# casinca/LLM-quest

Measured on AMD Instinct MI355X. Metric: img+tokens/sec fwd+bwd, ViT-B+Qwen3-0.6B VLM, 224px+512tok, higher is better.
Workload: dtype bf16; 1 GPU; BASELINE configs[3]: VLM early fusion, ViT-B/16 (frozen, fwd) + ffn adapter 768->3072->1024 + Qwen3-0.6B, 224x224 image + 512 text tokens (S=709), fwd+loss+bwd, no optimizer step; per_gpu_batch=160, global_batch=160, parallelism=dp1, text_mask=all ones, vision_tower_precision=bf16 MFMA operands, fp32 residual stream

## Files before the change

### llm_quest_amd/csrc/attention.hip

```cpp
#include "attn_common.h"

namespace {

template <int D>
__global__ __launch_bounds__(256, 2) void attn_fwd_kernel(int B, int S, int Hq, int Hkv, const bf16_t* __restrict__ q, int64_t ldq,
                                                          const bf16_t* __restrict__ k, int64_t ldk, const bf16_t* __restrict__ v,
                                                          int64_t ldv, bf16_t* __restrict__ o, int64_t ldo, float* __restrict__ lse,
                                                          const uint8_t* __restrict__ key_mask, int causal, float scale_log2) {
    using C = Cfg<D>;
    const int abl = causal >> 8;
    causal &= 0xff;
    __shared__ __attribute__((aligned(16))) char smem[4 * C::TILE];
    const int lane = threadIdx.x & 63;
    const int wave = __builtin_amdgcn_readfirstlane(threadIdx.x >> 6);
    const int nqb = (S + 127) / 128;
    const int vid = (abl >> 8) & 1 ? (int)blockIdx.x : xcd_chunked((int)blockIdx.x, (int)gridDim.x);
    const int qb = nqb - 1 - (vid % nqb);
    const int bh = vid / nqb;
    const int hq = bh % Hq, b = bh / Hq;
    const int hkv = hq / (Hq / Hkv);
    const int q0 = qb * 128;
    const int qg = q0 + wave * 32 + (lane & 31);
    const bool qvalid = qg < S;

// ... 636 lines not shown
                    }
                    dsv[e] = __builtin_amdgcn_exp2f(t) * (pacc[st][e] - dlt);
                    if constexpr (e % 2 == 1) dsw[st][e / 2] = pack_bf2(dsv[e - 1], dsv[e]);
                };
                static_for<PD>([&](auto g) { load(g); });
                static_for<NG>([&](auto gc) {
                    constexpr int g = gc.value;
                    load(std::integral_constant<int, g + PD>{});
                    if constexpr (g < 2 * NA) {
                        constexpr int st = g / NA, ks = (g % NA) / 2, which = g % 2;
                        if constexpr ((ATTN_ABL & 8) && ks > 0) {
                        } else if constexpr (which == 0) mfma_ownedB<OWNED, QF0 + 4 * ks, ks == 0>(sacc[st], f[g % RING]);
                        else mfma_ownedB<OWNED, OF0 + 4 * ks, ks == 0>(pacc[st], f[g % RING]);
                    } else if constexpr (!(ATTN_ABL & 4)) {
                        constexpr int h = g - 2 * NA, st = h / NC, sd = (h % NC) / DT, dt = h % DT;
                        const u32x4 w = {dsw[st][4 * sd], dsw[st][4 * sd + 1], dsw[st][4 * sd + 2], dsw[st][4 * sd + 3]};
                        constexpr int younger = NG - 1 - g < PD ? NG - 1 - g : PD;
                        mfma_owned<OWNED, 16 * dt>(tr_wait<2 * younger>(ft[g % RING]), __builtin_bit_cast(bf16x8, w));
                    }
                    if constexpr (g == NA) tiles_settle(sacc[0], pacc[0]);
                    if constexpr (g == 2 * NA) tiles_settle(sacc[1], pacc[1]);
                    if constexpr (g >= NA && g < 2 * NA) {
                        constexpr int m = g - NA, per = 16 / NA;
                        static_for<per>([&](auto i) { element(std::integral_constant<int, 0>{}, std::integral_constant<int, m * per + i.value>{}); });
                    } else if constexpr (g >= 2 * NA && g < 2 * NA + NC) {
                        constexpr int m = g - 2 * NA, per = 16 / NC;
                        static_for<per>([&](auto i) { element(std::integral_constant<int, 1>{}, std::integral_constant<int, m * per + i.value>{}); });
                    }
                    __builtin_amdgcn_sched_barrier(0);
                });
            };
            if (boundary) tile_body(std::true_type{});
            else tile_body(std::false_type{});
        }
        owned_settle<OWNED>();
        bf16_t* row = dq + ((int64_t)b * S + qg) * lddq + (int64_t)hq * D;
        static_for<DT * 4>([&](auto i) {
            constexpr int dt = i.value / 4, g4 = i.value % 4, r = 16 * dt + 4 * g4;
            const int d = dt * 32 + 8 * g4 + 4 * (lane >> 5);
            const u32x2 pk = {pack_bf2(owned_read<OWNED, r>() * scale, owned_read<OWNED, r + 1>() * scale),
                              pack_bf2(owned_read<OWNED, r + 2>() * scale, owned_read<OWNED, r + 3>() * scale)};
            if (qvalid && !(abl & 2)) *reinterpret_cast<u32x2*>(row + d) = pk;
        });
    }
}

template <int D, bool LEAN>
__global__ __launch_bounds__(256, 1) void attn_bwd_dkv_kernel(int B, int S, int Hq, int Hkv, const bf16_t* __restrict__ q, int64_t ldq,
                                                              const bf16_t* __restrict__ k, int64_t ldk, const bf16_t* __restrict__ v,
                                                              int64_t ldv, const bf16_t* __restrict__ d_o, int64_t lddo,
                                                              const float* __restrict__ lse, const float* __restrict__ delta,
                                                              bf16_t* __restrict__ dk, int64_t lddk, bf16_t* __restrict__ dv, int64_t lddv,
                                                              const uint8_t* __restrict__ key_mask, int causal, float scale, float scale_log2,
                                                              int bpw, bf16_t* __restrict__ ds_out) {
    using C = Cfg<D>;
    constexpr int KS = C::KS, DT = C::DT;
    constexpr int NA = 2 * KS, NC = 4 * DT, NG = 2 * NA + 2 * NC;
    constexpr int OWNED = 32 * DT + 8 * KS, DK0 = 16 * DT, KF0 = 32 * DT, VF0 = KF0 + 4 * KS;
    constexpr int RING = ATTN_RING, PD = ATTN_PD;
    constexpr bool UNI = C::UNI;
    constexpr int NIMG = UNI ? 2 : 4, NST = 3, STAGE = NIMG * C::TILE, PIECES = NIMG * C::PPW;
    constexpr int OIMG = (UNI ? 1 : 2) * C::TILE;
    const int abl = causal >> 8;
    causal &= 0xff;
    __shared__ __attribute__((aligned(16))) char smem[NST * STAGE + NST * 512];
    char* rowc = smem + NST * STAGE;
    const int lane = threadIdx.x & 63;
    const int wave = __builtin_amdgcn_readfirstlane(threadIdx.x >> 6);
    const int nkb = (S + 127) / 128, nchunk = (nkb + bpw - 1) / bpw;
    const int chunk = blockIdx.x % nchunk, bh = blockIdx.x / nchunk;
    const int hkv = bh % Hkv, b = bh / Hkv;
    const int rep = Hq / Hkv;
    const int kb_lo = chunk * bpw, kb_hi = min(nkb, kb_lo + bpw);
    const int nqt_all = (S + 63) / 64;
    auto qt0_of = [&](int kb) { return causal ? kb * 2 : 0; };

    int ikb = kb_lo, ih = 0, iq = 0, istage = 0;
    auto issue_next = [&]() -> bool {
        if (ikb < kb_hi && iq >= nqt_all - qt0_of(ikb)) { iq = 0; ++ih; }
        if (ikb < kb_hi && ih >= rep) { ih = 0; ++ikb; }
        if (ikb >= kb_hi) return false;
        const int hq = hkv * rep + ih;
        const int qt = qt0_of(ikb) + iq;
        char* st_ = smem + istage * STAGE;
        const bf16_t* qb_ = q + ((int64_t)b * S + (int64_t)qt * 64) * ldq + (int64_t)hq * D;
        const bf16_t* ob_ = d_o + ((int64_t)b * S + (int64_t)qt * 64) * lddo + (int64_t)hq * D;
        if constexpr (UNI) {
            dma_tile<D, IMG_UNI>(qb_, ldq, S - qt * 64, st_, wave, lane);
            dma_tile<D, IMG_UNI>(ob_, lddo, S - qt * 64, st_ + OIMG, wave, lane);
        } else {
            dma_tile<D, IMG_ROW>(qb_, ldq, S - qt * 64, st_, wave, lane);
            dma_tile<D, IMG_TR>(qb_, ldq, S - qt * 64, st_ + C::TILE, wave, lane);
            dma_tile<D, IMG_ROW>(ob_, lddo, S - qt * 64, st_ + OIMG, wave, lane);
            dma_tile<D, IMG_TR>(ob_, lddo, S - qt * 64, st_ + OIMG + C::TILE, wave, lane);
        }
        {
            const float* src = ((wave & 1) == 0 ? lse : delta) + ((int64_t)b * Hq + hq) * S + (int64_t)qt * 64;
            auto rsrc = __builtin_amdgcn_make_buffer_rsrc(const_cast<float*>(src), 0, 0x7fffffff, 0x00020000);
            const unsigned voff = qt * 64 + lane < S ? (unsigned)(lane * 4) : OOB;
            __builtin_amdgcn_raw_ptr_buffer_load_lds(rsrc, LDS_PTR(rowc + istage * 512 + (wave & 1) * 256), 4, voff, 0, 0, 0);
        }
        ++iq;
        istage = istage == NST - 1 ? 0 : istage + 1;
        return true;
    };
    [[maybe_unused]] const bool prof_on = threadIdx.x == 0;
    [[maybe_unused]] unsigned long long prof_acc[16] = {};
    [[maybe_unused]] const unsigned long long t_wg = PROF_T();
    int inflight = 0;
    inflight += issue_next();
    inflight += issue_next();

    const LaneOff<D> lo = lane_offsets<D>(lane);
    const unsigned lds0 = (unsigned)(unsigned long long)LDS_PTR(smem);
    int cstage = 0;
    int st1 = 0, st2 = 0;
    bf16x8 tk[KS], tv[KS];
    auto request_kv = [&](int kb_) {
        const int kg_ = kb_ * 128 + wave * 32 + (lane & 31);
        load_rows_frag<D>(k + (int64_t)b * S * ldk + (int64_t)hkv * D, ldk, kg_, kg_ < S, lane, tk);
        load_rows_frag<D>(v + (int64_t)b * S * ldv + (int64_t)hkv * D, ldv, kg_, kg_ < S, lane, tv);
    };
    if (kb_lo < kb_hi) request_kv(kb_lo);
    for (int kb = kb_lo; kb < kb_hi; ++kb) {
        [[maybe_unused]] const unsigned long long t_pro = PROF_T();
        const int k0 = kb * 128;
        const int kg = k0 + wave * 32 + (lane & 31);
        const bool kvalid = kg < S;
        const bool kreal = kvalid && (key_mask == nullptr || key_mask[(int64_t)b * S + kg] != 0);
        owned_zero<OWNED, 0, 32 * DT>();
        if constexpr (LEAN) {
#pragma unroll
            for (int ks = 0; ks < KS; ++ks) {
                u32x4 w = __builtin_bit_cast(u32x4, tk[ks]);
#pragma unroll
                for (int e = 0; e < 4; ++e) w[e] = pack_bf2(__uint_as_float(w[e] << 16) * scale_log2, __uint_as_float(w[e] & 0xffff0000u) * scale_log2);
                tk[ks] = __builtin_bit_cast(bf16x8, w);
            }
        }
        static_for<KS>([&](auto ks) { owned_write4<OWNED, KF0 + 4 * ks.value>(tk[ks.value]); });
        static_for<KS>([&](auto ks) { owned_write4<OWNED, VF0 + 4 * ks.value>(tv[ks.value]); });
        const int qt0 = qt0_of(kb);
        const int per_head = nqt_all - qt0;
        const int nit = per_head * rep;
        PROF_ADD(3, t_pro);
        int ch = 0, cq = -1;
        for (int it = 0; it < nit; ++it) {
            if (++cq == per_head) { cq = 0; ++ch; }
            [[maybe_unused]] const unsigned long long t_w = PROF_T();
            if (inflight >= 2) {
                if (st1 + st2 == 8) wait_vmcnt<PIECES + 1 + 8>();
                else if (st1 + st2 == 4) wait_vmcnt<PIECES + 1 + 4>();
                else wait_vmcnt<PIECES + 1>();
            } else wait_vmcnt<0>();
            st2 = st1;
            st1 = 0;
            PROF_ADD(1, t_w);
            [[maybe_unused]] const unsigned long long t_b = PROF_T();
            __builtin_amdgcn_s_barrier();
            PROF_ADD(6, t_b);
            --inflight;
            [[maybe_unused]] const unsigned long long t_i = PROF_T();
            if (!(abl & 1)) inflight += issue_next();
            PROF_ADD(7, t_i);
#if ATTN_ABL & 16
            struct BodyTimer {
                unsigned long long t0; bool on; unsigned long long* acc;
                __device__ ~BodyTimer() { if (on) { acc[2] += __builtin_readcyclecounter() - t0; acc[5] += 1; } }
            } body_timer{PROF_T(), prof_on, prof_acc};
#endif
            const int qt = qt0 + cq;
            const int qroff = cstage * STAGE, qtoff = UNI ? qroff : qroff + C::TILE, oroff = qroff + OIMG, otoff = UNI ? oroff : oroff + C::TILE;
            const float* rc = reinterpret_cast<const float*>(rowc + cstage * 512) + 4 * (lane >> 5);
            cstage = cstage == NST - 1 ? 0 : cstage + 1;
            if (causal && qt * 64 + 63 < k0 + wave * 32) continue;
            const bool boundary = (causal && qt * 64 < k0 + wave * 32 + 31) || (qt * 64 + 64 > S) || __any(!kreal);
            int vqx[KS], vox[KS], vqt[DT], vot[DT];
#pragma unroll
            for (int ks = 0; ks < KS; ++ks) {
                vqx[ks] = ((UNI ? lo.rowu : lo.row) + qroff) ^ (ks << 5);
                vox[ks] = ((UNI ? lo.rowu : lo.row) + oroff) ^ (ks << 5);
            }
#pragma unroll
            for (int dt = 0; dt < DT; ++dt) {
                vqt[dt] = (UNI ? lo.colu[dt] : lo.col[dt]) + qtoff;
                vot[dt] = (UNI ? lo.colu[dt] : lo.col[dt]) + otoff;
            }

            auto tile_body = [&](auto bc) {
                constexpr bool BOUNDARY = decltype(bc)::value;
                bf16x8 f[RING] = {};
                TrHalves ft[RING] = {};
                f32x16 sacc[2], pacc[2];
                unsigned pw[2][8] = {}, dsw[2][8] = {};
                float lsr[2][16], dlr[2][16], tt[2][16], pv[2][16], dsv[2][16];
                [[maybe_unused]] f32x16 linit[2], dinit[2];
                auto load = [&](auto gc) {
                    constexpr int g = gc.value;
                    if constexpr (ATTN_ABL & 1) return;
                    if constexpr (g < 2 * NA) {
                        constexpr int st = g / NA, ks = (g % NA) / 2, which = g % 2;
                        f[g % RING] = lds_frag(smem, which ? vox[ks] : vqx[ks], st * 32 * C::ROWB);
                    } else if constexpr (g < NG) {
                        constexpr int h = g - 2 * NA, st = h / NC, sd = (h % NC) / (2 * DT), dt = (h % (2 * DT)) / 2, which = h % 2;
                        constexpr int imm = (st * 32 + 16 * sd) * C::ROWB;
                        const int va = which ? vqt[dt] : vot[dt];
                        if constexpr (!(ATTN_ABL & 32)) tr_issue<imm, imm + 8 * C::ROWB>(ft[g % RING], lds0 + va, lds0 + (UNI ? va ^ 0x20 : va));
                    }
                };
                auto row_constants = [&](auto stc) {
                    constexpr int st = stc.value;
#pragma unroll
                    for (int g4 = 0; g4 < 4; ++g4) {
                        const f32x4 a = *reinterpret_cast<const f32x4*>(rc + st * 32 + 8 * g4);
                        const f32x4 c = *reinterpret_cast<const f32x4*>(rc + 64 + st * 32 + 8 * g4);
#pragma unroll
                        for (int e = 0; e < 4; ++e) {
                            if constexpr (LEAN) {
                                linit[st][4 * g4 + e] = a[e];
                                dinit[st][4 * g4 + e] = c[e];
                            } else {
                                lsr[st][4 * g4 + e] = a[e];
                                dlr[st][4 * g4 + e] = c[e];
                            }
                        }
                    }
                };
                auto stage = [&](auto stc, auto ec, auto kc) {
                    constexpr int st = stc.value, e = ec.value, k = kc.value;
                    if constexpr (e < 0 || e >= 16 || (ATTN_ABL & 2)) return;
                    else if constexpr (LEAN) {
                        if constexpr (k == 1 && BOUNDARY) {
                            const int qq = qt * 64 + st * 32 + acc_row(e, lane);
                            const bool masked = (causal && kg > qq) || !kreal || qq >= S;
                            sacc[st][e] = masked ? -INFINITY : sacc[st][e];
                            asm volatile("" : "+v"(sacc[st][e]));
                        } else if constexpr (k == 2) {
                            pv[st][e] = __builtin_amdgcn_exp2f(sacc[st][e]);
                            asm volatile("" : "+v"(pv[st][e]));
                        } else if constexpr (k == 3) {
                            dsv[st][e] = pacc[st][e] * pv[st][e];
                            if constexpr (e % 2 == 1) {
                                pw[st][e / 2] = pack_bf2(pv[st][e - 1], pv[st][e]);
                                dsw[st][e / 2] = pack_bf2(dsv[st][e - 1], dsv[st][e]);
                                asm volatile("" : "+v"(pw[st][e / 2]), "+v"(dsw[st][e / 2]));
                            } else {
                                asm volatile("" : "+v"(dsv[st][e]));
                            }
                        }
                    } else if constexpr (k == 0) {
                        lsr[st][e] *= LOG2E;
                        asm volatile("" : "+v"(lsr[st][e]));
                    } else if constexpr (k == 1) {
                        float t = fmaf(sacc[st][e], scale_log2, -lsr[st][e]);
                        if constexpr (BOUNDARY) {
                            const int qq = qt * 64 + st * 32 + acc_row(e, lane);
                            const bool masked = (causal && kg > qq) || !kreal || qq >= S;
                            t = masked ? -INFINITY : t;
                        }
                        tt[st][e] = t;
                        asm volatile("" : "+v"(tt[st][e]));
                    } else if constexpr (k == 2) {
                        pv[st][e] = __builtin_amdgcn_exp2f(tt[st][e]);
                        dsv[st][e] = pacc[st][e] - dlr[st][e];
                        asm volatile("" : "+v"(pv[st][e]), "+v"(dsv[st][e]));
                    } else {
                        dsv[st][e] *= pv[st][e];
                        if constexpr (e % 2 == 1) {
                            pw[st][e / 2] = pack_bf2(pv[st][e - 1], pv[st][e]);
                            dsw[st][e / 2] = pack_bf2(dsv[st][e - 1], dsv[st][e]);
                            asm volatile("" : "+v"(pw[st][e / 2]), "+v"(dsw[st][e / 2]));
                        } else {
                            asm volatile("" : "+v"(dsv[st][e]));
                        }
                    }
                };
                auto b_step = [&](auto stc, auto mc, auto perc) {
                    constexpr int m = mc.value, PER = perc.value;
                    if constexpr (m >= 0 && m < 16 / PER + 3)
                        static_for<4>([&](auto kc) {
                            static_for<PER>([&](auto i) { stage(stc, std::integral_constant<int, (m - kc.value) * PER + i.value>{}, kc); });
                        });
                };
                if constexpr (LEAN) row_constants(std::integral_constant<int, 0>{});
                static_for<PD>([&](auto g) { load(g); });
                [[maybe_unused]] unsigned long long t_seg = PROF_T();
                static_for<NG>([&](auto gc) {
                    constexpr int g = gc.value;
#if ATTN_ABL & 16
                    if constexpr (g == NA || g == 2 * NA || g == 2 * NA + NC) {
                        if (prof_on) { const unsigned long long now = __builtin_readcyclecounter(); prof_acc[8 + (g == NA ? 0 : g == 2 * NA ? 1 : 2)] += now - t_seg; t_seg = now; }
                    }
#endif
                    if constexpr (!LEAN && g == NA - 1) row_constants(std::integral_constant<int, 0>{});
                    if constexpr (LEAN && g == NA - 4) row_constants(std::integral_constant<int, 1>{});
                    load(std::integral_constant<int, g + PD>{});
                    if constexpr (g < 2 * NA) {
                        constexpr int st = g / NA, ks = (g % NA) / 2, which = g % 2;
                        if constexpr ((ATTN_ABL & 8) && ks > 0) {
                        } else if constexpr (LEAN && ks == 0) {
                            if constexpr (which == 0) mfma_ownedB_init<OWNED, KF0>(sacc[st], f[g % RING], linit[st]);
                            else mfma_ownedB_init<OWNED, VF0>(pacc[st], f[g % RING], dinit[st]);
                        } else if constexpr (which == 0) mfma_ownedB<OWNED, KF0 + 4 * ks, ks == 0>(sacc[st], f[g % RING]);
                        else mfma_ownedB<OWNED, VF0 + 4 * ks, ks == 0>(pacc[st], f[g % RING]);
                    } else if constexpr (!(ATTN_ABL & 4)) {
                        constexpr int h = g - 2 * NA, st = h / NC, sd = (h % NC) / (2 * DT), dt = (h % (2 * DT)) / 2, which = h % 2;
                        constexpr int younger = NG - 1 - g < PD ? NG - 1 - g : PD;
                        const bf16x8 fa = tr_wait<2 * younger>(ft[g % RING]);
                        if constexpr (which == 0) {
                            const u32x4 w = {pw[st][4 * sd], pw[st][4 * sd + 1], pw[st][4 * sd + 2], pw[st][4 * sd + 3]};
                            mfma_owned<OWNED, 16 * dt, false>(fa, __builtin_bit_cast(bf16x8, w));
                        } else {
                            const u32x4 w = {dsw[st][4 * sd], dsw[st][4 * sd + 1], dsw[st][4 * sd + 2], dsw[st][4 * sd + 3]};
                            mfma_owned<OWNED, DK0 + 16 * dt, false>(fa, __builtin_bit_cast(bf16x8, w));
                        }
                    }
                    if constexpr (g == NA) tiles_settle(sacc[0], pacc[0]);
                    if constexpr (g == 2 * NA) tiles_settle(sacc[1], pacc[1]);
                    static_assert(16 % NA == 0 && 16 % NC == 0 && 16 / (16 / NA) + 3 <= NA + NC / 2 && 16 / (16 / NC) + 3 <= NC + NC / 2, "B phase does not fit its gaps");
                    b_step(std::integral_constant<int, 0>{}, std::integral_constant<int, g - NA>{}, std::integral_constant<int, 16 / NA>{});
                    b_step(std::integral_constant<int, 1>{}, std::integral_constant<int, g - 2 * NA>{}, std::integral_constant<int, 16 / NC>{});
                    if constexpr (!LEAN && g == 2 * NA - 1) row_constants(std::integral_constant<int, 1>{});
                    __builtin_amdgcn_sched_barrier(0);
                });
                PROF_ADD(11, t_seg);
                if (ds_out) {
                    const int hq_ = hkv * rep + ch;
                    const int nqb_ = (S + 127) / 128;
                    char* blk = reinterpret_cast<char*>(ds_out) + ((((int64_t)b * Hq + hq_) * (2 * nqb_) + qt) * 2 * (4 * nqb_) + (kb * 4 + wave)) * 2048 + lane * 16;
                    static_for<4>([&](auto i) {
                        constexpr int st = i.value / 2, c2 = i.value % 2;
                        const u32x4 w4 = {dsw[st][4 * c2], dsw[st][4 * c2 + 1], dsw[st][4 * c2 + 2], dsw[st][4 * c2 + 3]};
                        *reinterpret_cast<u32x4*>(blk + (int64_t)st * (4 * nqb_) * 2048 + c2 * 1024) = w4;
                    });
                }
            };
            if (boundary) tile_body(std::true_type{});
            else tile_body(std::false_type{});
            st1 = ds_out != nullptr ? 4 : 0;
        }
        [[maybe_unused]] const unsigned long long t_epi = PROF_T();
        owned_settle<OWNED>();
        if (kb + 1 < kb_hi) request_kv(kb + 1);
        bf16_t* krow = dk + ((int64_t)b * S + kg) * lddk + (int64_t)hkv * D + 8 * (lane >> 5);
        bf16_t* vrow = dv + ((int64_t)b * S + kg) * lddv + (int64_t)hkv * D + 8 * (lane >> 5);
        static_for<DT * 2>([&](auto i) {
            constexpr int dt = i.value / 2, gp = i.value % 2, rv = 16 * dt + 8 * gp, rk = DK0 + rv;
            const unsigned ka0 = pack_bf2(owned_read<OWNED, rk>() * scale, owned_read<OWNED, rk + 1>() * scale), ka1 = pack_bf2(owned_read<OWNED, rk + 2>() * scale, owned_read<OWNED, rk + 3>() * scale);
            const unsigned kb0 = pack_bf2(owned_read<OWNED, rk + 4>() * scale, owned_read<OWNED, rk + 5>() * scale), kb1 = pack_bf2(owned_read<OWNED, rk + 6>() * scale, owned_read<OWNED, rk + 7>() * scale);
            const unsigned va0 = pack_bf2(owned_read<OWNED, rv>(), owned_read<OWNED, rv + 1>()), va1 = pack_bf2(owned_read<OWNED, rv + 2>(), owned_read<OWNED, rv + 3>());
            const unsigned vb0 = pack_bf2(owned_read<OWNED, rv + 4>(), owned_read<OWNED, rv + 5>()), vb1 = pack_bf2(owned_read<OWNED, rv + 6>(), owned_read<OWNED, rv + 7>());
            const auto k0s = __builtin_amdgcn_permlane32_swap(ka0, kb0, false, false), k1s = __builtin_amdgcn_permlane32_swap(ka1, kb1, false, false);
            const auto v0s = __builtin_amdgcn_permlane32_swap(va0, vb0, false, false), v1s = __builtin_amdgcn_permlane32_swap(va1, vb1, false, false);
            const u32x4 wk = {k0s[0], k1s[0], k0s[1], k1s[1]}, wv = {v0s[0], v1s[0], v0s[1], v1s[1]};
            if (kvalid && !(abl & 2)) {
                *reinterpret_cast<u32x4*>(krow + dt * 32 + 16 * gp) = wk;
                *reinterpret_cast<u32x4*>(vrow + dt * 32 + 16 * gp) = wv;
            }
        });
        PROF_ADD(4, t_epi);
    }
    PROF_ADD(0, t_wg);
#if ATTN_ABL & 16
    if (prof_on)
        for (int i = 0; i < 16; ++i) atomicAdd(&g_prof[i], prof_acc[i]);
#endif
}

struct QkFuse {
    const bf16_t* qkv;
    int64_t ldqkv;
    const bf16_t* qw;
    const float* cosT;
    const float* sinT;
    const int32_t* pos;
    const float* rstd;
    int rstd_heads;
    bf16_t* dqkv;
    int64_t lddqkv;
    float* dwp;
    const bf16_t* cs16;
};
__device__ __forceinline__ void unpack4(const u32x2 v, float (&o)[4]) {
    o[0] = __uint_as_float(v[0] << 16);
    o[1] = __uint_as_float(v[0] & 0xffff0000u);
    o[2] = __uint_as_float(v[1] << 16);
    o[3] = __uint_as_float(v[1] & 0xffff0000u);
}
__device__ __forceinline__ float round_bf(float x) { return bf2f(f2bf(x)); }

#ifndef DQ_ABL
#define DQ_ABL 0
#endif
#if DQ_ABL & 16
__device__ unsigned long long g_dq_prof[32];
#define DQ_T() __builtin_readcyclecounter()
#define DQ_MARK(i) do { const unsigned long long now_ = __builtin_readcyclecounter(); dqp[i] += now_ - dq_t; dq_t = now_; } while (0)
#else
#define DQ_T() 0ull
#define DQ_MARK(i) do { } while (0)
#endif
template <int D, bool FUSE>
__global__ __launch_bounds__(256, 2) void attn_bwd_dq_spill_kernel(int B, int S, int Hq, int Hkv, const bf16_t* __restrict__ k, int64_t ldk,
                                                                   const bf16_t* __restrict__ ds, bf16_t* __restrict__ dq, int64_t lddq,
                                                                   int causal, float scale, QkFuse f) {
    using C = Cfg<D>;
    constexpr int DT = C::DT, DSW = 4096;
    constexpr int KST = 2, DST = 3, DS_BASE = KST * C::TILE, DS_STAGE = 4 * DSW;
    __shared__ __attribute__((aligned(16))) char smem[KST * C::TILE + DST * DS_STAGE];
    const int lane = threadIdx.x & 63;
    const int wave = __builtin_amdgcn_readfirstlane(threadIdx.x >> 6);
    const int nqb = (S + 127) / 128;
    const int vid = xcd_chunked((int)blockIdx.x, (int)gridDim.x);
    int qb, bh;
    heavy_first(vid, nqb, B * Hq, ATTN_HEAD_GROUP, qb, bh);
    const int hq = bh % Hq, b = bh / Hq;
    const int hkv = hq / (Hq / Hkv);
    const int q0 = qb * 128;
    const int qw = q0 + wave * 32;
    const int qg = qw + (lane & 31);
    const int ntiles_all = (S + 63) / 64;
    const int ntiles = causal ? min(ntiles_all, (q0 + 127) / 64 + 1) : ntiles_all;
    const bf16_t* kbase = k + (int64_t)b * S * ldk + (int64_t)hkv * D;
    const char* sblk = reinterpret_cast<const char*>(ds) + (((((int64_t)b * Hq + hq) * (2 * nqb) + 2 * qb + (wave >> 1)) * 2 + (wave & 1)) * (4 * nqb)) * 2048;
    auto srsrc = __builtin_amdgcn_make_buffer_rsrc(const_cast<char*>(sblk), 0, 0x7fffffff, 0x00020000);
    const unsigned unit = (unsigned)(lane ^ ((lane >> 5) << 2)) * 16;
    auto fetched = [&](int kgrp) { return !(causal && kgrp * 32 > qw + 31) && kgrp * 32 < S; };
    auto issue_k = [&](int kt) {
        if (!((DQ_ABL & 2) && kt > 0)) dma_tile<D, IMG_TR>(kbase + (int64_t)kt * 64 * ldk, ldk, S - kt * 64, smem + (kt % KST) * C::TILE, wave, lane);
    };
    auto issue_ds = [&](int kt) {
        char* mine = smem + DS_BASE + (kt % DST) * DS_STAGE + wave * DSW;
#pragma unroll
        for (int half = 0; half < 2; ++half) {
            const bool live = fetched(2 * kt + half) && kt < ntiles && !((DQ_ABL & 1) && kt > 0);
            const unsigned o0 = live ? (unsigned)((2 * kt + half) * 2048) + unit : OOB;
            const unsigned o1 = live ? (unsigned)((2 * kt + half) * 2048 + 1024) + unit : OOB;
            __builtin_amdgcn_raw_ptr_buffer_load_lds(srsrc, LDS_PTR(mine + half * 2048), 16, o0, 0, 0, 0);
            __builtin_amdgcn_raw_ptr_buffer_load_lds(srsrc, LDS_PTR(mine + half * 2048 + 1024), 16, o1, 0, 0, 0);
        }
    };
    const LaneOff<D> lok = lane_offsets<D>(lane);
    const int g = lane >> 4, q4 = (lane >> 2) & 3, p = lane & 3;
    const unsigned scol = (unsigned)((g & 1) * 1024 + ((((p & 1) * 32 + 4 * (g >> 1) + q4) ^ ((p & 1) << 2)) * 16) + (p >> 1) * 8) + DS_BASE + wave * DSW;
    const unsigned lds0 = (unsigned)(unsigned long long)LDS_PTR(smem);
    f32x16 acc[DT];
#pragma unroll
    for (int i = 0; i < DT; ++i)
#pragma unroll
        for (int e = 0; e < 16; ++e) acc[i][e] = 0.f;
    [[maybe_unused]] unsigned long long dqp[8] = {};
    [[maybe_unused]] unsigned long long dq_t = DQ_T();
    [[maybe_unused]] const unsigned long long dq_t0 = dq_t;
    [[maybe_unused]] int pos_pre[4] = {0, 0, 0, 0};
    if constexpr (FUSE) {
#pragma unroll
        for (int it = 0; it < 4; ++it) {
            const int qrow = q0 + (int)(threadIdx.x >> 3) + 32 * it;
            pos_pre[it] = f.pos[(int64_t)b * S + (qrow < S ? qrow : S - 1)];
        }
    }
    issue_ds(0);
    issue_k(0);
    issue_ds(1);
    for (int kt = 0; kt < ntiles; ++kt) {
        wait_vmcnt<4>();
        DQ_MARK(0);
        __builtin_amdgcn_s_barrier();
        DQ_MARK(1);
        if (kt + 1 < ntiles) issue_k(kt + 1);
        else issue_ds(ntiles);
        issue_ds(kt + 2);
        DQ_MARK(2);
        const unsigned kimg = lds0 + (kt % KST) * C::TILE, simg = lds0 + (kt % DST) * DS_STAGE + scol;
        static_for<2>([&](auto hc) {
            constexpr int half = hc.value;
            if (!fetched(2 * kt + half)) return;
            if constexpr (DQ_ABL & 4) return;
            TrHalves bs[2], ak[2][DT];
            static_for<2>([&](auto sc) {
// ... 343 lines not shown
    if (D == 128)
        hipLaunchKernelGGL(attn_fwd_kernel<128>, dim3((unsigned)grid), dim3(256), 0, s, B, S, Hq, Hkv, (const bf16_t*)q, ldq, (const bf16_t*)k, ldk, (const bf16_t*)v, ldv, (bf16_t*)o, ldo, lse, key_mask, causal, sl2);
    else
        hipLaunchKernelGGL(attn_fwd_kernel<64>, dim3((unsigned)grid), dim3(256), 0, s, B, S, Hq, Hkv, (const bf16_t*)q, ldq, (const bf16_t*)k, ldk, (const bf16_t*)v, ldv, (bf16_t*)o, ldo, lse, key_mask, causal, sl2);
    MI355_LAUNCH_CHECK("mi355_attn_fwd");
    return 0;
}

static int64_t attn_bwd_ds_bytes(int B, int S, int Hq) {
    const int64_t nqb = (S + 127) / 128;
    return (int64_t)B * Hq * nqb * nqb * 128 * 128 * 2;
}
extern "C" int64_t mi355_attn_bwd_workspace_bytes(int B, int S, int Hq, int D) {
    if (D != 128 || B <= 0 || S <= 0 || Hq <= 0) return 0;
    return attn_bwd_ds_bytes(B, S, Hq) + 2 * (((int64_t)B * Hq * S * 4 + 15) & ~(int64_t)15);
}

extern "C" int mi355_attn_bwd_ws(int B, int S, int Hq, int Hkv, int D, const void* q, int64_t ldq, const void* k, int64_t ldk,
                                 const void* v, int64_t ldv, const void* o, int64_t ldo, const void* d_o, int64_t lddo,
                                 const float* lse, float* delta, void* dq, int64_t lddq, void* dk, int64_t lddk, void* dv,
                                 int64_t lddv, const uint8_t* key_mask, int causal, float scale, void* workspace, int64_t workspace_bytes,
                                 void* stream);

extern "C" int mi355_attn_bwd(int B, int S, int Hq, int Hkv, int D, const void* q, int64_t ldq, const void* k, int64_t ldk,
                              const void* v, int64_t ldv, const void* o, int64_t ldo, const void* d_o, int64_t lddo,
                              const float* lse, float* delta, void* dq, int64_t lddq, void* dk, int64_t lddk, void* dv,
                              int64_t lddv, const uint8_t* key_mask, int causal, float scale, void* stream) {
    return mi355_attn_bwd_ws(B, S, Hq, Hkv, D, q, ldq, k, ldk, v, ldv, o, ldo, d_o, lddo, lse, delta, dq, lddq, dk, lddk, dv, lddv, key_mask, causal, scale,
                             nullptr, 0, stream);
}

static int attn_bwd_impl(int B, int S, int Hq, int Hkv, int D, const void* q, int64_t ldq, const void* k, int64_t ldk,
                         const void* v, int64_t ldv, const void* o, int64_t ldo, const void* d_o, int64_t lddo,
                         const float* lse, float* delta, void* dq, int64_t lddq, void* dk, int64_t lddk, void* dv,
                         int64_t lddv, const uint8_t* key_mask, int causal, float scale, void* workspace, int64_t workspace_bytes,
                         void* stream, const QkFuse* fuse) {
    if (check_common("mi355_attn_bwd", B, S, Hq, Hkv, D)) return 1;
    const bool delta_ready = (causal & MI355_ATTN_DELTA_READY) != 0;
    causal &= ~MI355_ATTN_DELTA_READY;
    if (fuse) {
        dq = const_cast<void*>(q);
        lddq = ldq;
    }
    MI355_REQUIRE(q && k && v && o && d_o && lse && delta && dq && dk && dv, "mi355_attn_bwd: null pointer");
    MI355_REQUIRE(((ldq | ldk | ldv | ldo | lddo | lddq | lddk | lddv) & 7) == 0, "mi355_attn_bwd: leading dimensions must be multiples of 8");
    MI355_REQUIRE((((uintptr_t)q | (uintptr_t)k | (uintptr_t)v | (uintptr_t)o | (uintptr_t)d_o | (uintptr_t)dq | (uintptr_t)dk | (uintptr_t)dv) & 15) == 0,
                  "mi355_attn_bwd: operands and gradients must be 16-byte aligned");
    hipStream_t s = (hipStream_t)stream;
    const float sl2 = scale * LOG2E;
    const int64_t items = (int64_t)B * S * ((Hq + 512 / D - 1) / (512 / D));
    const int dgrid = (int)((items + 3) / 4 > 8192 ? 8192 : (items + 3) / 4);
    const int nblk = (S + 127) / 128;
    const int bpw_q = (int64_t)B * Hq >= 512 ? nblk : 1;
    const int bpw_k = (int64_t)B * Hkv >= 512 ? nblk : 1;
    const int64_t gq = (int64_t)B * Hq * ((nblk + bpw_q - 1) / bpw_q), gk = (int64_t)B * Hkv * ((nblk + bpw_k - 1) / bpw_k);
    MI355_REQUIRE(S <= 64 * ATTN_MAX_TILES, "mi355_attn_bwd: S must be <= %d", 64 * ATTN_MAX_TILES);
    MI355_REQUIRE(gq < 0x7fffffffLL, "mi355_attn_bwd: grid too large");
    const bool spill = D == 128 && workspace != nullptr && !((causal >> 8) & 1024);
    MI355_REQUIRE(!fuse || spill, "mi355_attn_bwd_qnorm: head_dim 128 and a workspace (the one-product dQ pass) are required");
    if (spill) {
        MI355_REQUIRE(workspace_bytes >= mi355_attn_bwd_workspace_bytes(B, S, Hq, D), "mi355_attn_bwd_ws: workspace of %lld bytes, %lld needed",
                      (long long)workspace_bytes, (long long)mi355_attn_bwd_workspace_bytes(B, S, Hq, D));
        MI355_REQUIRE(((uintptr_t)workspace & 15) == 0, "mi355_attn_bwd_ws: workspace must be 16-byte aligned");
    }
    MI355_REQUIRE(!delta_ready || spill, "mi355_attn_bwd: MI355_ATTN_DELTA_READY needs the workspace form (head_dim 128)");
    bf16_t* ds_ws = spill ? (bf16_t*)workspace : nullptr;
    float* nl2 = spill ? (float*)((char*)workspace + attn_bwd_ds_bytes(B, S, Hq)) : nullptr;
    float* ndl = spill ? (float*)((char*)nl2 + (((int64_t)B * Hq * S * 4 + 15) & ~(int64_t)15)) : nullptr;
#define BWD_LAUNCH(DD)                                                                                                              \
    if (!delta_ready)                                                                                                               \
        hipLaunchKernelGGL(attn_delta_kernel<DD>, dim3(dgrid), dim3(256), 0, s, B, S, Hq, (const bf16_t*)o, ldo, (const bf16_t*)d_o, lddo, delta, lse, nl2, ndl); \
    if (spill && DD == 128)                                                                                                         \
        hipLaunchKernelGGL((attn_bwd_dkv_kernel<128, true>), dim3((unsigned)gk), dim3(256), 0, s, B, S, Hq, Hkv, (const bf16_t*)q, ldq, (const bf16_t*)k, ldk, \
                           (const bf16_t*)v, ldv, (const bf16_t*)d_o, lddo, nl2, ndl, (bf16_t*)dk, lddk, (bf16_t*)dv, lddv, key_mask, causal, scale, sl2, bpw_k, ds_ws); \
    else                                                                                                                             \
        hipLaunchKernelGGL((attn_bwd_dkv_kernel<DD, false>), dim3((unsigned)gk), dim3(256), 0, s, B, S, Hq, Hkv, (const bf16_t*)q, ldq, (const bf16_t*)k, ldk, \
                           (const bf16_t*)v, ldv, (const bf16_t*)d_o, lddo, lse, delta, (bf16_t*)dk, lddk, (bf16_t*)dv, lddv, key_mask, causal, scale, sl2, bpw_k, ds_ws); \
    if (!spill)                                                                                                                      \
        hipLaunchKernelGGL(attn_bwd_dq_kernel<DD>, dim3((unsigned)gq), dim3(256), 0, s, B, S, Hq, Hkv, (const bf16_t*)q, ldq, (const bf16_t*)k, ldk,  \
                           (const bf16_t*)v, ldv, (const bf16_t*)d_o, lddo, lse, delta, (bf16_t*)dq, lddq, key_mask, causal, scale, sl2, bpw_q);
    if (D == 128) {
        BWD_LAUNCH(128)
        if (spill && fuse)
            hipLaunchKernelGGL((attn_bwd_dq_spill_kernel<128, true>), dim3((unsigned)((int64_t)B * Hq * nblk)), dim3(256), 0, s, B, S, Hq, Hkv, (const bf16_t*)k, ldk,
                               (const bf16_t*)ds_ws, (bf16_t*)nullptr, (int64_t)0, causal & 0xff, scale, *fuse);
        else if (spill)
            hipLaunchKernelGGL((attn_bwd_dq_spill_kernel<128, false>), dim3((unsigned)((int64_t)B * Hq * nblk)), dim3(256), 0, s, B, S, Hq, Hkv, (const bf16_t*)k, ldk,
                               (const bf16_t*)ds_ws, (bf16_t*)dq, lddq, causal & 0xff, scale, QkFuse{});
    } else {
        BWD_LAUNCH(64)
    }
#undef BWD_LAUNCH
    MI355_LAUNCH_CHECK("mi355_attn_bwd");
    return 0;
}

extern "C" int64_t mi355_attn_bwd_workspace_rowconst_offset(int B, int S, int Hq, int D, int which) {
    if (D != 128 || B <= 0 || S <= 0 || Hq <= 0 || which < 0 || which > 1) return -1;
    const int64_t first = attn_bwd_ds_bytes(B, S, Hq);
    return which == 0 ? first : first + (((int64_t)B * Hq * S * 4 + 15) & ~(int64_t)15);
}

extern "C" int mi355_attn_bwd_ws(int B, int S, int Hq, int Hkv, int D, const void* q, int64_t ldq, const void* k, int64_t ldk,
                                 const void* v, int64_t ldv, const void* o, int64_t ldo, const void* d_o, int64_t lddo,
                                 const float* lse, float* delta, void* dq, int64_t lddq, void* dk, int64_t lddk, void* dv,
                                 int64_t lddv, const uint8_t* key_mask, int causal, float scale, void* workspace, int64_t workspace_bytes,
                                 void* stream) {
    return attn_bwd_impl(B, S, Hq, Hkv, D, q, ldq, k, ldk, v, ldv, o, ldo, d_o, lddo, lse, delta, dq, lddq, dk, lddk, dv, lddv, key_mask, causal, scale, workspace,
                         workspace_bytes, stream, nullptr);
}

extern "C" int64_t mi355_attn_bwd_qnorm_partials(int B, int S, int Hq) { return (int64_t)B * Hq * ((S + 127) / 128); }

extern "C" int mi355_attn_bwd_qnorm(int B, int S, int Hq, int Hkv, int D, const void* q, int64_t ldq, const void* k, int64_t ldk, const void* v, int64_t ldv,
                                    const void* o, int64_t ldo, const void* d_o, int64_t lddo, const float* lse, float* delta, void* dk, int64_t lddk,
                                    void* dv, int64_t lddv, const uint8_t* key_mask, int causal, float scale, void* workspace, int64_t workspace_bytes,
                                    const void* qkv, int64_t ldqkv, const void* q_weight, const float* cos, const float* sin, const int32_t* pos,
                                    const float* rstd, int rstd_heads, void* dqkv, int64_t lddqkv, float* dqw_partial, const void* rope_cs16, void* stream) {
    MI355_REQUIRE(D == 128, "mi355_attn_bwd_qnorm: head_dim must be 128 (got %d)", D);
    MI355_REQUIRE(qkv && q_weight && cos && sin && pos && rstd && dqkv && dqw_partial && workspace, "mi355_attn_bwd_qnorm: null pointer");
    MI355_REQUIRE(rstd_heads >= Hq && ldqkv >= (int64_t)Hq * D && lddqkv >= (int64_t)Hq * D && ((ldqkv | lddqkv) & 3) == 0,
                  "mi355_attn_bwd_qnorm: qkv / dqkv rows must hold the query heads (8-byte aligned pitches), rstd one column per head");
    MI355_REQUIRE((((uintptr_t)qkv | (uintptr_t)dqkv | (uintptr_t)q_weight) & 7) == 0 && (((uintptr_t)cos | (uintptr_t)sin) & 15) == 0,
                  "mi355_attn_bwd_qnorm: qkv / dqkv / weight 8-byte aligned, cos / sin 16-byte aligned");
    MI355_REQUIRE(!rope_cs16 || ((uintptr_t)rope_cs16 & 15) == 0, "mi355_attn_bwd_qnorm: rope_cs16 must be 16-byte aligned");
    const QkFuse f{(const bf16_t*)qkv, ldqkv, (const bf16_t*)q_weight, cos, sin, pos, rstd, rstd_heads, (bf16_t*)dqkv, lddqkv, dqw_partial, (const bf16_t*)rope_cs16};
    return attn_bwd_impl(B, S, Hq, Hkv, D, q, ldq, k, ldk, v, ldv, o, ldo, d_o, lddo, lse, delta, nullptr, 0, dk, lddk, dv, lddv, key_mask, causal, scale, workspace,
                         workspace_bytes, stream, &f);
}
```

### llm_quest_amd/csrc/attn_common.h

```cpp
#pragma once
#include <type_traits>

#include "common.h"

namespace {

constexpr float MASK_T = -2.0e38f;
constexpr float LOG2E = 1.4426950408889634f;
constexpr float LN2 = 0.6931471805599453f;
constexpr unsigned OOB = 0x80000000u;
constexpr int ATTN_MAX_TILES = 512;

template <int D>
struct Cfg {
    static constexpr int ROWB = D * 2;
    static constexpr int CH = ROWB / 16;
    static constexpr int KS = D / 16;
    static constexpr int DT = D / 32;
    static constexpr int TILE = 64 * ROWB;
    static constexpr int RPP = 1024 / ROWB;
    static constexpr int PPW = TILE / 1024 / 4;
    static constexpr bool UNI = (D == 128);
};

// ... 174 lines not shown
__device__ __forceinline__ void static_for(F&& f) {
    if constexpr (N > 0) {
        static_for<N - 1>(f);
        f(std::integral_constant<int, N - 1>{});
    }
}
template <int OWNED, int OFF, bool NOP = true>
__device__ __forceinline__ void mfma_owned(const bf16x8& a, const bf16x8& b) {
    static_assert(OFF % 16 == 0 && OFF + 16 <= OWNED, "tile outside the owned range");
    constexpr int R0 = 256 - OWNED + OFF;
    if constexpr (NOP) OWNED_ASM(OWNED, "s_nop 1\n\tv_mfma_f32_32x32x16_bf16 a[%c2:%c3], %0, %1, a[%c2:%c3]" ::"v"(a), "v"(b), "i"(R0), "i"(R0 + 15));
    else OWNED_ASM(OWNED, "v_mfma_f32_32x32x16_bf16 a[%c2:%c3], %0, %1, a[%c2:%c3]" ::"v"(a), "v"(b), "i"(R0), "i"(R0 + 15));
}
template <int OWNED, int OFF, bool FIRST>
__device__ __forceinline__ void mfma_ownedB(f32x16& acc, const bf16x8& a) {
    static_assert(OFF % 4 == 0 && OFF + 4 <= OWNED, "operand outside the owned range");
    constexpr int R0 = 256 - OWNED + OFF;
    if constexpr (FIRST) OWNED_ASM(OWNED, "v_mfma_f32_32x32x16_bf16 %0, %1, a[%c2:%c3], 0" : "=&v"(acc) : "v"(a), "i"(R0), "i"(R0 + 3));
    else OWNED_ASM(OWNED, "v_mfma_f32_32x32x16_bf16 %0, %1, a[%c2:%c3], %0" : "+v"(acc) : "v"(a), "i"(R0), "i"(R0 + 3));
}
template <int OWNED, int OFF>
__device__ __forceinline__ void mfma_ownedB_init(f32x16& acc, const bf16x8& a, const f32x16& init) {
    static_assert(OFF % 4 == 0 && OFF + 4 <= OWNED, "operand outside the owned range");
    constexpr int R0 = 256 - OWNED + OFF;
    OWNED_ASM(OWNED, "v_mfma_f32_32x32x16_bf16 %0, %1, a[%c3:%c4], %2" : "=&v"(acc) : "v"(a), "v"(init), "i"(R0), "i"(R0 + 3));
}
__device__ __forceinline__ void tiles_settle(f32x16& x, f32x16& y) { asm volatile("s_nop 15\n\ts_nop 3" : "+v"(x), "+v"(y)); }
template <int OWNED, int OFF, int COUNT>
__device__ __forceinline__ void owned_zero() {
    static_for<COUNT>([&](auto r) { OWNED_ASM(OWNED, "v_accvgpr_write_b32 a[%c0], 0" ::"i"(256 - OWNED + OFF + r.value)); });
}
template <int OWNED, int OFF>
__device__ __forceinline__ void owned_write4(const bf16x8& v) {
    const u32x4 w = __builtin_bit_cast(u32x4, v);
    OWNED_ASM(OWNED, "v_accvgpr_write_b32 a[%c4], %0\n\tv_accvgpr_write_b32 a[%c5], %1\n\tv_accvgpr_write_b32 a[%c6], %2\n\tv_accvgpr_write_b32 a[%c7], %3"
              ::"v"(w[0]), "v"(w[1]), "v"(w[2]), "v"(w[3]), "i"(256 - OWNED + OFF), "i"(256 - OWNED + OFF + 1), "i"(256 - OWNED + OFF + 2), "i"(256 - OWNED + OFF + 3));
}
template <int OWNED>
__device__ __forceinline__ void owned_settle() { OWNED_ASM(OWNED, "s_nop 15\n\ts_nop 3" ::); }
template <int OWNED, int R>
__device__ __forceinline__ float owned_read() {
    float x;
    asm volatile("v_accvgpr_read_b32 %0, a[%c1]" : "=v"(x) : "i"(256 - OWNED + R));
    return x;
}

__device__ __forceinline__ int acc_row(int e, int lane) { return (e & 3) + 8 * (e >> 2) + 4 * (lane >> 5); }

__device__ __forceinline__ int xcd_chunked(int b, int n) {
    const int xcd = b & 7, q = n >> 3, r = n & 7;
    return (xcd < r ? xcd * (q + 1) : r * (q + 1) + (xcd - r) * q) + (b >> 3);
}

}
```

### llm_quest_amd/fingerprint.py

```python

import hashlib
import json
import os
import re

_HERE = os.path.dirname(os.path.abspath(__file__))
EVIDENCE_ROUND = "r06"
FILES = ("attention.hip", "attn_common.h", "elementwise.hip", "gemm.hip", "norm_rope.hip", "common.h")
_FLAG_LINES = re.compile(r"^(CXXFLAGS|ARCH|FLAGS_(?:attention|elementwise|gemm|norm_rope))\s*\??=")


def compile_flags():
    out = []
    with open(os.path.join(_HERE, "csrc", "Makefile")) as fh:
        for line in fh:
            if _FLAG_LINES.match(line):
                out.append(" ".join(line.split()))
    return "\n".join(out)


def kernel_sources_sha():
    h = hashlib.sha256()
    for n in FILES:
        h.update(n.encode())
        with open(os.path.join(_HERE, "csrc", n), "rb") as fh:
            h.update(fh.read())
    h.update(compile_flags().encode())
    return h.hexdigest()[:16]


def all_sources_sha():
    h = hashlib.sha256()
    d = os.path.join(_HERE, "csrc")
    for n in sorted(f for f in os.listdir(d) if f.endswith((".hip", ".h")) and not f.startswith("_")):
        h.update(n.encode())
        with open(os.path.join(d, n), "rb") as fh:
            h.update(fh.read())
    with open(os.path.join(d, "Makefile")) as fh:
        h.update("\n".join(" ".join(line.split()) for line in fh if re.match(r"^(CXXFLAGS|ARCH|FLAGS_\w+)\s*\??=", line)).encode())
    return h.hexdigest()[:16]


def library_sha():
    with open(os.path.join(_HERE, "libmi355vlm.so"), "rb") as fh:
        return hashlib.sha256(fh.read()).hexdigest()[:16]


def collection_stamp(evidence_dir):
    with open(os.path.join(evidence_dir, "stamp.json")) as f:
        return json.load(f)


if __name__ == "__main__":
    import sys

    print(json.dumps({"kernel_sources_sha": kernel_sources_sha(), "all_sources_sha": all_sources_sha(), "library_sha": library_sha(), "git_sha": sys.argv[1] if len(sys.argv) > 1 else "unknown",
                      "per_gpu_batch": int(sys.argv[2]) if len(sys.argv) > 2 else None}))
```

Measured before the change: 191,800 img+tok/s.

## Pair causal key blocks per dK/dV workgroup and add half-tile path

```diff
diff --git a/llm_quest_amd/csrc/attention.hip b/llm_quest_amd/csrc/attention.hip
--- a/llm_quest_amd/csrc/attention.hip
+++ b/llm_quest_amd/csrc/attention.hip
@@ -712,7 +712,7 @@
                                                               const float* __restrict__ lse, const float* __restrict__ delta,
                                                               bf16_t* __restrict__ dk, int64_t lddk, bf16_t* __restrict__ dv, int64_t lddv,
                                                               const uint8_t* __restrict__ key_mask, int causal, float scale, float scale_log2,
-                                                              int bpw, bf16_t* __restrict__ ds_out) {
+                                                              int paired, bf16_t* __restrict__ ds_out) {
     using C = Cfg<D>;
     constexpr int KS = C::KS, DT = C::DT;
     constexpr int NA = 2 * KS, NC = 4 * DT, NG = 2 * NA + 2 * NC;
@@ -727,21 +727,21 @@
     char* rowc = smem + NST * STAGE;
     const int lane = threadIdx.x & 63;
     const int wave = __builtin_amdgcn_readfirstlane(threadIdx.x >> 6);
-    const int nkb = (S + 127) / 128, nchunk = (nkb + bpw - 1) / bpw;
-    const int chunk = blockIdx.x % nchunk, bh = blockIdx.x / nchunk;
+    const int nkb = (S + 127) / 128, npw = dkv_workgroups(nkb, paired != 0);
+    const int vid = xcd_chunked((int)blockIdx.x, (int)gridDim.x);
+    const int bh = vid / npw;
     const int hkv = bh % Hkv, b = bh / Hkv;
     const int rep = Hq / Hkv;
-    const int kb_lo = chunk * bpw, kb_hi = min(nkb, kb_lo + bpw);
     const int nqt_all = (S + 63) / 64;
-    auto qt0_of = [&](int kb) { return causal ? kb * 2 : 0; };
-
-    int ikb = kb_lo, ih = 0, iq = 0, istage = 0;
+
+    DkvWalk iw;
+    iw.start(vid - bh * npw, nkb, nqt_all, rep, causal, paired != 0);
+    DkvWalk cw = iw;
+    int istage = 0;
     auto issue_next = [&]() -> bool {
-        if (ikb < kb_hi && iq >= nqt_all - qt0_of(ikb)) { iq = 0; ++ih; }
-        if (ikb < kb_hi && ih >= rep) { ih = 0; ++ikb; }
-        if (ikb >= kb_hi) return false;
-        const int hq = hkv * rep + ih;
-        const int qt = qt0_of(ikb) + iq;
+        if (iw.done()) return false;
+        const int hq = hkv * rep + iw.h;
+        const int qt = iw.qt;
         char* st_ = smem + istage * STAGE;
         const bf16_t* qb_ = q + ((int64_t)b * S + (int64_t)qt * 64) * ldq + (int64_t)hq * D;
         const bf16_t* ob_ = d_o + ((int64_t)b * S + (int64_t)qt * 64) * lddo + (int64_t)hq * D;
@@ -760,7 +760,7 @@
             const unsigned voff = qt * 64 + lane < S ? (unsigned)(lane * 4) : OOB;
             __builtin_amdgcn_raw_ptr_buffer_load_lds(rsrc, LDS_PTR(rowc + istage * 512 + (wave & 1) * 256), 4, voff, 0, 0, 0);
         }
-        ++iq;
+        iw.next();
         istage = istage == NST - 1 ? 0 : istage + 1;
         return true;
     };
@@ -781,9 +781,10 @@
         load_rows_frag<D>(k + (int64_t)b * S * ldk + (int64_t)hkv * D, ldk, kg_, kg_ < S, lane, tk);
         load_rows_frag<D>(v + (int64_t)b * S * ldv + (int64_t)hkv * D, ldv, kg_, kg_ < S, lane, tv);
     };
-    if (kb_lo < kb_hi) request_kv(kb_lo);
-    for (int kb = kb_lo; kb < kb_hi; ++kb) {
+    request_kv(cw.kb);
+    while (!cw.done()) {
         [[maybe_unused]] const unsigned long long t_pro = PROF_T();
+        const int kb = cw.kb;
         const int k0 = kb * 128;
         const int kg = k0 + wave * 32 + (lane & 31);
         const bool kvalid = kg < S;
@@ -800,17 +801,17 @@
         }
         static_for<KS>([&](auto ks) { owned_write4<OWNED, KF0 + 4 * ks.value>(tk[ks.value]); });
         static_for<KS>([&](auto ks) { owned_write4<OWNED, VF0 + 4 * ks.value>(tv[ks.value]); });
-        const int qt0 = qt0_of(kb);
-        const int per_head = nqt_all - qt0;
-        const int nit = per_head * rep;
+        const int nit = cw.tiles();
         PROF_ADD(3, t_pro);
-        int ch = 0, cq = -1;
         for (int it = 0; it < nit; ++it) {
-            if (++cq == per_head) { cq = 0; ++ch; }
+            const int qt = cw.qt, ch = cw.h;
+            cw.next();
             [[maybe_unused]] const unsigned long long t_w = PROF_T();
             if (inflight >= 2) {
                 if (st1 + st2 == 8) wait_vmcnt<PIECES + 1 + 8>();
+                else if (st1 + st2 == 6) wait_vmcnt<PIECES + 1 + 6>();
                 else if (st1 + st2 == 4) wait_vmcnt<PIECES + 1 + 4>();
+                else if (st1 + st2 == 2) wait_vmcnt<PIECES + 1 + 2>();
                 else wait_vmcnt<PIECES + 1>();
             } else wait_vmcnt<0>();
             st2 = st1;
@@ -829,7 +830,6 @@
                 __device__ ~BodyTimer() { if (on) { acc[2] += __builtin_readcyclecounter() - t0; acc[5] += 1; } }
             } body_timer{PROF_T(), prof_on, prof_acc};
 #endif
-            const int qt = qt0 + cq;
             const int qroff = cstage * STAGE, qtoff = UNI ? qroff : qroff + C::TILE, oroff = qroff + OIMG, otoff = UNI ? oroff : oroff + C::TILE;
             const float* rc = reinterpret_cast<const float*>(rowc + cstage * 512) + 4 * (lane >> 5);
             cstage = cstage == NST - 1 ? 0 : cstage + 1;
@@ -847,8 +847,10 @@
                 vot[dt] = (UNI ? lo.colu[dt] : lo.col[dt]) + otoff;
             }
 
-            auto tile_body = [&](auto bc) {
-                constexpr bool BOUNDARY = decltype(bc)::value;
+            auto tile_body = [&](auto bc, auto hc) {
+                constexpr bool BOUNDARY = decltype(bc)::value, HALF = decltype(hc)::value;
+                static_assert(!HALF || BOUNDARY, "a half tile ends the sequence: it is a boundary tile");
+                constexpr int NGL = HALF ? 2 * NA + NC : NG;
                 bf16x8 f[RING] = {};
                 TrHalves ft[RING] = {};
                 f32x16 sacc[2], pacc[2];
@@ -858,6 +860,7 @@
                 auto load = [&](auto gc) {
                     constexpr int g = gc.value;
                     if constexpr (ATTN_ABL & 1) return;
+                    if constexpr (HALF && ((g >= NA && g < 2 * NA) || g >= NGL)) return;
                     if constexpr (g < 2 * NA) {
                         constexpr int st = g / NA, ks = (g % NA) / 2, which = g % 2;
                         f[g % RING] = lds_frag(smem, which ? vox[ks] : vqx[ks], st * 32 * C::ROWB);
@@ -953,9 +956,10 @@
                     }
 #endif
                     if constexpr (!LEAN && g == NA - 1) row_constants(std::integral_constant<int, 0>{});
-                    if constexpr (LEAN && g == NA - 4) row_constants(std::integral_constant<int, 1>{});
+                    if constexpr (LEAN && !HALF && g == NA - 4) row_constants(std::integral_constant<int, 1>{});
                     load(std::integral_constant<int, g + PD>{});
-                    if constexpr (g < 2 * NA) {
+                    if constexpr (HALF && ((g >= NA && g < 2 * NA) || g >= NGL)) {
+                    } else if constexpr (g < 2 * NA) {
                         constexpr int st = g / NA, ks = (g % NA) / 2, which = g % 2;
                         if constexpr ((ATTN_ABL & 8) && ks > 0) {
                         } else if constexpr (LEAN && ks == 0) {
@@ -965,7 +969,7 @@
                         else mfma_ownedB<OWNED, VF0 + 4 * ks, ks == 0>(pacc[st], f[g % RING]);
                     } else if constexpr (!(ATTN_ABL & 4)) {
                         constexpr int h = g - 2 * NA, st = h / NC, sd = (h % NC) / (2 * DT), dt = (h % (2 * DT)) / 2, which = h % 2;
-                        constexpr int younger = NG - 1 - g < PD ? NG - 1 - g : PD;
+                        constexpr int younger = NGL - 1 - g < PD ? NGL - 1 - g : PD;
                         const bf16x8 fa = tr_wait<2 * younger>(ft[g % RING]);
                         if constexpr (which == 0) {
                             const u32x4 w = {pw[st][4 * sd], pw[st][4 * sd + 1], pw[st][4 * sd + 2], pw[st][4 * sd + 3]};
@@ -976,11 +980,11 @@
                         }
                     }
                     if constexpr (g == NA) tiles_settle(sacc[0], pacc[0]);
-                    if constexpr (g == 2 * NA) tiles_settle(sacc[1], pacc[1]);
+                    if constexpr (!HALF && g == 2 * NA) tiles_settle(sacc[1], pacc[1]);
                     static_assert(16 % NA == 0 && 16 % NC == 0 && 16 / (16 / NA) + 3 <= NA + NC / 2 && 16 / (16 / NC) + 3 <= NC + NC / 2, "B phase does not fit its gaps");
                     b_step(std::integral_constant<int, 0>{}, std::integral_constant<int, g - NA>{}, std::integral_constant<int, 16 / NA>{});
-                    b_step(std::integral_constant<int, 1>{}, std::integral_constant<int, g - 2 * NA>{}, std::integral_constant<int, 16 / NC>{});
-                    if constexpr (!LEAN && g == 2 * NA - 1) row_constants(std::integral_constant<int, 1>{});
+                    if constexpr (!HALF) b_step(std::integral_constant<int, 1>{}, std::integral_constant<int, g - 2 * NA>{}, std::integral_constant<int, 16 / NC>{});
+                    if constexpr (!LEAN && !HALF && g == 2 * NA - 1) row_constants(std::integral_constant<int, 1>{});
                     __builtin_amdgcn_sched_barrier(0);
                 });
                 PROF_ADD(11, t_seg);
@@ -988,20 +992,22 @@
                     const int hq_ = hkv * rep + ch;
                     const int nqb_ = (S + 127) / 128;
                     char* blk = reinterpret_cast<char*>(ds_out) + ((((int64_t)b * Hq + hq_) * (2 * nqb_) + qt) * 2 * (4 * nqb_) + (kb * 4 + wave)) * 2048 + lane * 16;
-                    static_for<4>([&](auto i) {
+                    static_for<HALF ? 2 : 4>([&](auto i) {
                         constexpr int st = i.value / 2, c2 = i.value % 2;
                         const u32x4 w4 = {dsw[st][4 * c2], dsw[st][4 * c2 + 1], dsw[st][4 * c2 + 2], dsw[st][4 * c2 + 3]};
                         *reinterpret_cast<u32x4*>(blk + (int64_t)st * (4 * nqb_) * 2048 + c2 * 1024) = w4;
                     });
                 }
             };
-            if (boundary) tile_body(std::true_type{});
-            else tile_body(std::false_type{});
-            st1 = ds_out != nullptr ? 4 : 0;
+            const bool half = S - qt * 64 <= 32;
+            if (half) tile_body(std::true_type{}, std::true_type{});
+            else if (boundary) tile_body(std::true_type{}, std::false_type{});
+            else tile_body(std::false_type{}, std::false_type{});
+            st1 = ds_out == nullptr ? 0 : half ? 2 : 4;
         }
         [[maybe_unused]] const unsigned long long t_epi = PROF_T();
         owned_settle<OWNED>();
-        if (kb + 1 < kb_hi) request_kv(kb + 1);
+        if (!cw.done()) request_kv(cw.kb);
         bf16_t* krow = dk + ((int64_t)b * S + kg) * lddk + (int64_t)hkv * D + 8 * (lane >> 5);
         bf16_t* vrow = dv + ((int64_t)b * S + kg) * lddv + (int64_t)hkv * D + 8 * (lane >> 5);
         static_for<DT * 2>([&](auto i) {
@@ -1085,7 +1091,7 @@
     const char* sblk = reinterpret_cast<const char*>(ds) + (((((int64_t)b * Hq + hq) * (2 * nqb) + 2 * qb + (wave >> 1)) * 2 + (wave & 1)) * (4 * nqb)) * 2048;
     auto srsrc = __builtin_amdgcn_make_buffer_rsrc(const_cast<char*>(sblk), 0, 0x7fffffff, 0x00020000);
     const unsigned unit = (unsigned)(lane ^ ((lane >> 5) << 2)) * 16;
-    auto fetched = [&](int kgrp) { return !(causal && kgrp * 32 > qw + 31) && kgrp * 32 < S; };
+    auto fetched = [&](int kgrp) { return !(causal && kgrp * 32 > qw + 31) && kgrp * 32 < S && qw < S; };
     auto issue_k = [&](int kt) {
         if (!((DQ_ABL & 2) && kt > 0)) dma_tile<D, IMG_TR>(kbase + (int64_t)kt * 64 * ldk, ldk, S - kt * 64, smem + (kt % KST) * C::TILE, wave, lane);
     };
@@ -1535,10 +1541,10 @@
     const int dgrid = (int)((items + 3) / 4 > 8192 ? 8192 : (items + 3) / 4);
     const int nblk = (S + 127) / 128;
     const int bpw_q = (int64_t)B * Hq >= 512 ? nblk : 1;
-    const int bpw_k = (int64_t)B * Hkv >= 512 ? nblk : 1;
-    const int64_t gq = (int64_t)B * Hq * ((nblk + bpw_q - 1) / bpw_q), gk = (int64_t)B * Hkv * ((nblk + bpw_k - 1) / bpw_k);
+    const int pair_k = (int64_t)B * Hkv >= 512 ? 1 : 0;
+    const int64_t gq = (int64_t)B * Hq * ((nblk + bpw_q - 1) / bpw_q), gk = (int64_t)B * Hkv * dkv_workgroups(nblk, pair_k != 0);
     MI355_REQUIRE(S <= 64 * ATTN_MAX_TILES, "mi355_attn_bwd: S must be <= %d", 64 * ATTN_MAX_TILES);
-    MI355_REQUIRE(gq < 0x7fffffffLL, "mi355_attn_bwd: grid too large");
+    MI355_REQUIRE(gq < 0x7fffffffLL && gk < 0x7fffffffLL, "mi355_attn_bwd: grid too large");
     const bool spill = D == 128 && workspace != nullptr && !((causal >> 8) & 1024);
     MI355_REQUIRE(!fuse || spill, "mi355_attn_bwd_qnorm: head_dim 128 and a workspace (the one-product dQ pass) are required");
     if (spill) {
@@ -1555,10 +1561,10 @@
         hipLaunchKernelGGL(attn_delta_kernel<DD>, dim3(dgrid), dim3(256), 0, s, B, S, Hq, (const bf16_t*)o, ldo, (const bf16_t*)d_o, lddo, delta, lse, nl2, ndl); \
     if (spill && DD == 128)                                                                                                         \
         hipLaunchKernelGGL((attn_bwd_dkv_kernel<128, true>), dim3((unsigned)gk), dim3(256), 0, s, B, S, Hq, Hkv, (const bf16_t*)q, ldq, (const bf16_t*)k, ldk, \
-                           (const bf16_t*)v, ldv, (const bf16_t*)d_o, lddo, nl2, ndl, (bf16_t*)dk, lddk, (bf16_t*)dv, lddv, key_mask, causal, scale, sl2, bpw_k, ds_ws); \
+                           (const bf16_t*)v, ldv, (const bf16_t*)d_o, lddo, nl2, ndl, (bf16_t*)dk, lddk, (bf16_t*)dv, lddv, key_mask, causal, scale, sl2, pair_k, ds_ws); \
     else                                                                                                                             \
         hipLaunchKernelGGL((attn_bwd_dkv_kernel<DD, false>), dim3((unsigned)gk), dim3(256), 0, s, B, S, Hq, Hkv, (const bf16_t*)q, ldq, (const bf16_t*)k, ldk, \
-                           (const bf16_t*)v, ldv, (const bf16_t*)d_o, lddo, lse, delta, (bf16_t*)dk, lddk, (bf16_t*)dv, lddv, key_mask, causal, scale, sl2, bpw_k, ds_ws); \
+                           (const bf16_t*)v, ldv, (const bf16_t*)d_o, lddo, lse, delta, (bf16_t*)dk, lddk, (bf16_t*)dv, lddv, key_mask, causal, scale, sl2, pair_k, ds_ws); \
     if (!spill)                                                                                                                      \
         hipLaunchKernelGGL(attn_bwd_dq_kernel<DD>, dim3((unsigned)gq), dim3(256), 0, s, B, S, Hq, Hkv, (const bf16_t*)q, ldq, (const bf16_t*)k, ldk,  \
                            (const bf16_t*)v, ldv, (const bf16_t*)d_o, lddo, lse, delta, (bf16_t*)dq, lddq, key_mask, causal, scale, sl2, bpw_q);
diff --git a/llm_quest_amd/csrc/attn_common.h b/llm_quest_amd/csrc/attn_common.h
--- a/llm_quest_amd/csrc/attn_common.h
+++ b/llm_quest_amd/csrc/attn_common.h
@@ -250,4 +250,31 @@
     return (xcd < r ? xcd * (q + 1) : r * (q + 1) + (xcd - r) * q) + (b >> 3);
 }
 
-}
+__host__ __device__ inline bool dkv_descending(int kb, int nkb) { return 2 * kb < nkb; }
+__host__ __device__ inline int dkv_first_tile(int kb, int causal) { return causal ? 2 * kb : 0; }
+__host__ __device__ inline int dkv_workgroups(int nkb, bool paired) { return paired ? (nkb + 1) / 2 : nkb; }
+struct DkvWalk {
+    int nkb, nqt, rep, causal, paired;
+    int kb, qt, h;
+    __host__ __device__ void enter(int kb_) {
+        kb = kb_;
+        h = 0;
+        qt = dkv_descending(kb_, nkb) ? nqt - 1 : dkv_first_tile(kb_, causal);
+    }
+    __host__ __device__ void start(int i, int nkb_, int nqt_, int rep_, int causal_, bool paired_) {
+        nkb = nkb_, nqt = nqt_, rep = rep_, causal = causal_, paired = paired_;
+        enter(i);
+    }
+    __host__ __device__ bool done() const { return kb < 0; }
+    __host__ __device__ int tiles() const { return (nqt - dkv_first_tile(kb, causal)) * rep; }
+    __host__ __device__ void next() {
+        if (++h < rep) return;
+        h = 0;
+        const bool down = dkv_descending(kb, nkb);
+        if (qt != (down ? dkv_first_tile(kb, causal) : nqt - 1)) qt += down ? -1 : 1;
+        else if (paired && 2 * kb < nkb - 1) enter(nkb - 1 - kb);
+        else kb = -1;
+    }
+};
+
+}
diff --git a/llm_quest_amd/fingerprint.py b/llm_quest_amd/fingerprint.py
--- a/llm_quest_amd/fingerprint.py
+++ b/llm_quest_amd/fingerprint.py
@@ -5,7 +5,7 @@
 import re
 
 _HERE = os.path.dirname(os.path.abspath(__file__))
-EVIDENCE_ROUND = "r06"
+EVIDENCE_ROUND = "r07"
 FILES = ("attention.hip", "attn_common.h", "elementwise.hip", "gemm.hip", "norm_rope.hip", "common.h")
 _FLAG_LINES = re.compile(r"^(CXXFLAGS|ARCH|FLAGS_(?:attention|elementwise|gemm|norm_rope))\s*\??=")
 
```

Result: no change. 192,600 img+tok/s, median of 6 (+0.4%).
